# sapeirone/EgoPack

Hardware: AMD Instinct MI355X
Metric: clip-seqs/sec training, AR+LTA+PNR multi-task (higher is better)
Workload: dtype bf16; 1 GPU; MTL pre-train AR+LTA+PNR (BASELINE config 3): per GPU B=64 seqs/task x T=32 nodes, 3x1536-d Omnivore-shaped features, H=1024, TRN hidden 1024 (dropout 0.5), depth 3, k=1, Adam; graph mode, fused backbone pass; global_batch=192, parallelism=dp1, trainable_params=25003272, capture=one graph, input=resident in HBM before the timed region, master_weights=f32, mode=bf16, activations=bf16

## Files before the change

### egopack_amd/csrc/gemm.hip

```cpp
#include <type_traits>

#include "common.h"

namespace egk {

typedef __attribute__((ext_vector_type(4))) float f32x4;
typedef __attribute__((ext_vector_type(8))) __bf16 bf16x8;
typedef unsigned short bf16_t;

constexpr int BM = 128, BN = 128, ROWB = 128;
constexpr int NTHREADS = 256;

constexpr int MAXSRC = 6;
struct GemmArgs {
    int M, N;
    int nsrc;
    int K[MAXSRC];
    const void* A[MAXSRC];
    const void* B[MAXSRC];
    long long lda[MAXSRC], ldb[MAXSRC];
    int a_vec, b_vec;
    void* C;
    long long ldc;
    int c_vec, c_bf16;
    int accumulate, act;
    float alpha;
    const float* bias;
    const void* residual;
    long long ldr;
    int r_vec, r_bf16;
    int splitk;
    float* ws;
    int tiles_m, tiles_n;
    int group_m;
    float* dbias;
    float* ws_bias;
    int rows_epilogue;
    int st_mode, st_nseg;
    const int* st_seg_ptr;
    double* st_ws;
    const void* st_x;
    long long st_ldx;
    const float* st_stats;
    const float* st_w;
    const float* st_b;
    float st_slope;
};

__device__ __forceinline__ void tile_of_virtual(const GemmArgs& g, int v, int& z, int& tm, int& tn) {
    const int tiles = g.tiles_m * g.tiles_n;
    z = v / tiles;
    const int t = v - z * tiles;
    const int gsz = g.group_m * g.tiles_n;
    const int grp = t / gsz, first = grp * g.group_m;
    const int rows = min(g.group_m, g.tiles_m - first);
    const int rr = t - grp * gsz;
    tm = first + rr % rows;
    tn = rr / rows;
}
__device__ __forceinline__ void tile_of(const GemmArgs& g, int bid, int& z, int& tm, int& tn) {
    const int tiles = g.tiles_m * g.tiles_n, nwg = tiles * g.splitk;
    const int xcd = bid & 7, q = nwg >> 3, r = nwg & 7;
    const int v = (xcd < r ? xcd * (q + 1) : r * (q + 1) + (xcd - r) * q) + (bid >> 3);
    z = v / tiles;
    const int t = v - z * tiles;
    const int gsz = g.group_m * g.tiles_n;
    const int grp = t / gsz, first = grp * g.group_m;
    const int rows = min(g.group_m, g.tiles_m - first);
    const int rr = t - grp * gsz;
    tm = first + rr % rows;
    tn = rr / rows;
}

template <int KT>
__device__ __forceinline__ void source_of(const GemmArgs& g, int t, int& src, int& tt) {
    src = 0;
    tt = t;
    while (src + 1 < g.nsrc) {
        const int n = (g.K[src] + KT - 1) / KT;
// ... 370 lines not shown
                const float* xp = (const float*)g.st_x + (long long)m * g.st_ldx + n;
                const float4 x0 = *reinterpret_cast<const float4*>(xp), x1 = *reinterpret_cast<const float4*>(xp + 4);
                xv[0] = x0.x; xv[1] = x0.y; xv[2] = x0.z; xv[3] = x0.w; xv[4] = x1.x; xv[5] = x1.y; xv[6] = x1.z; xv[7] = x1.w;
            }
            float a1 = 0.f, a2 = 0.f;
#pragma unroll
            for (int t = 0; t < 8; ++t) {
                const float xh = (xv[t] - mu) * ri;
                const float pre = xh * lw[t] + lb[t];
                const float dxh = o[t] * (pre > 0.f ? 1.f : g.st_slope) * lw[t];
                a1 += dxh;
                a2 += dxh * xh;
            }
            sa[rel][0] += a1;
            sa[rel][1] += a2;
        }
    }
    if constexpr (ST) if (st_mode) {
        __shared__ double st_red_static[MBW == 1 ? 4 : 1][4];
        double (*st_red)[4] = st_red_static;
        if constexpr (MBW == 2) st_red = reinterpret_cast<double (*)[4]>(lds + 32 * NI * MBW * 512);
        double v4[4] = {(double)sa[0][0], (double)sa[0][1], (double)sa[1][0], (double)sa[1][1]};
#pragma unroll
        for (int q = 0; q < 4; ++q)
#pragma unroll
            for (int o_ = 32; o_ > 0; o_ >>= 1) v4[q] += __shfl_xor(v4[q], o_, 64);
        if ((tid & 63) == 0) {
#pragma unroll
            for (int q = 0; q < 4; ++q) st_red[tid >> 6][q] = v4[q];
        }
        __syncthreads();
        if (tid < g.st_nseg * 2) {
            const int sg = tid >> 1, k = tid & 1, rel = sg - s0;
            double t_ = 0.0;
            if (rel == 0 || rel == 1) {
                t_ = (st_red[0][rel * 2 + k] + st_red[1][rel * 2 + k]) + (st_red[2][rel * 2 + k] + st_red[3][rel * 2 + k]);
                if constexpr (MBW == 2)
                    t_ += (st_red[4][rel * 2 + k] + st_red[5][rel * 2 + k]) + (st_red[6][rel * 2 + k] + st_red[7][rel * 2 + k]);
            }
            g.st_ws[((long long)st_tile * g.st_nseg + sg) * 2 + k] = t_;
        }
    }
}

template <bool BF16C, bool TA, bool TB, typename AT, typename BT>
__global__ __launch_bounds__(NTHREADS) void gemm_kernel(const GemmArgs g) {
    __shared__ __attribute__((aligned(16))) unsigned char lds[2 * BM * ROWB];
    unsigned char* ldsA = lds;
    unsigned char* ldsB = lds + BM * ROWB;
    constexpr int KT = BF16C ? 64 : 32;
    constexpr bool A16 = sizeof(AT) == 2, B16 = sizeof(BT) == 2;

    const int nwg = g.tiles_m * g.tiles_n;
    int bid = blockIdx.x;
    {
        const int xcd = bid & 7, q = nwg >> 3, r = nwg & 7;
        bid = (xcd < r ? xcd * (q + 1) : r * (q + 1) + (xcd - r) * q) + (bid >> 3);
    }
    const int tm = bid / g.tiles_n, tn = bid % g.tiles_n;
    const int m0 = tm * BM, n0 = tn * BN;

    const int nkt = total_tiles(g, KT);
    const int z = blockIdx.y;
    const int per = (nkt + g.splitk - 1) / g.splitk;
    const int t_begin = z * per, t_end = min(nkt, t_begin + per);

// ... 173 lines not shown
            const int L = wall - WG;
            OperandCursor<TRA, PA> la;
            OperandCursor<TRB, PB> lb;
            int lsrc = -1;
            auto lissue = [&](int i, int stage) {
                const int t = t_begin + i;
                int src, tt;
                source_of<KT>(g, t, src, tt);
                if (src != lsrc) {
                    const int k0 = tt * KT;
                    la.init((const bf16_t*)g.A[src], g.lda[src], g.M, m0, k0, L * PA, lane, 1);
                    lb.init((const bf16_t*)g.B[src], g.ldb[src], g.N, n0, k0, L * PB, lane, 1);
                    lsrc = src;
                }
                unsigned char* sbase = ring + stage * STAGE;
                la.issue(sbase, L * PA);
                lb.issue(sbase + IMG_A, L * PB);
            };
#pragma unroll
            for (int p = 0; p < NSTAGE - 1; ++p)
                if (p < nt) lissue(p, p);
            for (int it = 0; it < rounds; ++it) {
                const int later = min(NSTAGE - 2, nt - 1 - it);
                if (later >= 2) asm volatile("s_waitcnt vmcnt(%0)" ::"n"(2 * (PA + PB)) : "memory");
                else if (later == 1) asm volatile("s_waitcnt vmcnt(%0)" ::"n"(PA + PB) : "memory");
                else asm volatile("s_waitcnt vmcnt(0)" ::: "memory");
                __builtin_amdgcn_s_barrier();
                if (it + NSTAGE - 1 < nt) lissue(it + NSTAGE - 1, (it + NSTAGE - 1) % NSTAGE);
            }
            return;
        }
    }

    f32x4 acc[NI][4];
#pragma unroll
    for (int i = 0; i < NI; ++i)
#pragma unroll
        for (int j = 0; j < 4; ++j) acc[i][j] = f32x4{0.f, 0.f, 0.f, 0.f};

    const unsigned lds_base = (unsigned)(size_t)(lds_void_t*)ring;
    const unsigned rm_sw = (unsigned)((lg ^ ((lr >> 1) & 7)) << 4);
    const unsigned a_rm = (unsigned)((wm * 16 * NI + lr) * ROWB) + rm_sw;
    const unsigned b_rm = (unsigned)((wn * 64 + lr) * ROWB) + rm_sw;
    const int tq = (lane & 15) >> 2, tp = lane & 3;
    const unsigned tr_row = (unsigned)((8 * lg + tq) * 256 + (tp & 1) * 8);
    const unsigned tr_f = (unsigned)(2 * tq + 8 * (lg & 1));
    unsigned a_tr[4], b_tr[4];
#pragma unroll
    for (int i = 0; i < 4; ++i) {
        a_tr[i] = (unsigned)((wm >> 1) * IMG) + tr_row + ((((unsigned)((wm & 1) * 8 + 2 * i + (tp >> 1))) ^ tr_f) << 4);
        b_tr[i] = tr_row + ((((unsigned)(wn * 8 + 2 * i + (tp >> 1))) ^ tr_f) << 4);
    }

    const bool do_bias = TRA && g.dbias != nullptr && tn == 0;
    float bsum[8] = {0.f, 0.f, 0.f, 0.f, 0.f, 0.f, 0.f, 0.f};
    const int bcc = tid & 15, bkg = (tid & 255) >> 4;
    const int bsub = MB == 2 ? (tid >> 8) : 0;

    uint4 a0[4], a1[4], b0[4], b1[4];
    if constexpr (LW == 0) {
#pragma unroll
        for (int p = 0; p < NSTAGE - 1; ++p)
            if (p < nt) issue(p, p);
    }
    for (int it = 0; it < rounds; ++it) {
        if constexpr (LW == 0) {
// ... 100 lines not shown
                    const unsigned wv[4] = {bz[r].x, bz[r].y, bz[r].z, bz[r].w};
#pragma unroll
                    for (int e = 0; e < 4; ++e) {
                        bsum[2 * e] += __uint_as_float(wv[e] << 16);
                        bsum[2 * e + 1] += __uint_as_float(wv[e] & 0xffff0000u);
                    }
                }
            }
        }
    }
#ifdef EGK_GEMM_STAMPS
    const unsigned long long ps_loop = __builtin_amdgcn_s_memtime();
#endif
    if constexpr (TRA) {
        if (g.dbias != nullptr && tn == 0) {
            __syncthreads();
            float* red = reinterpret_cast<float*>(lds);
            const int slot = MB == 2 ? bsub : grp;
#pragma unroll
            for (int e = 0; e < 8; ++e) red[(slot * 16 + bkg) * 128 + bcc * 8 + e] = bsum[e];
            __syncthreads();
            if (tid < 128 * MB && m0 + tid < g.M) {
                const int q0 = MB == 2 ? (tid >> 7) * 16 : 0, nq = MB == 2 ? 16 : 16 * KG;
                float t = 0.f;
                for (int q = 0; q < nq; ++q) t += red[(q0 + q) * 128 + (tid & 127)];
                if (g.splitk > 1) g.ws_bias[(long long)z * g.M + m0 + tid] = t;
                else g.dbias[m0 + tid] += t;
            }
            __syncthreads();
        }
    }
    if constexpr (KG == 1) {
        if constexpr (MB == 1) {
            if (epilogue_rows_ok(g)) gemm_epilogue_rows<NI>(g, acc, lds, m0, n0, wm, wn, lr, lg, z, tid, tm * g.tiles_n + tn);
            else gemm_epilogue<NI, 4>(g, acc, m0, n0, wm * 16 * NI, wn * 64, lr, lg, z);
        } else if constexpr (NI == 3) {
            static_assert(NSTAGE * STAGE >= 192 * 512 + 256, "the rows epilogue stages the whole tile (+ the wave partials) in the ring");
            if (epilogue_rows_ok(g)) gemm_epilogue_rows<NI, true, 2>(g, acc, lds, m0, n0, wm, wn, lr, lg, z, tid, tm * g.tiles_n + tn);
            else gemm_epilogue<NI, 4>(g, acc, m0, n0, wm * 16 * NI, wn * 64, lr, lg, z);
        } else {
            gemm_epilogue<NI, 4>(g, acc, m0, n0, wm * 16 * NI, wn * 64, lr, lg, z);
        }
    } else if constexpr (NI == 4 || NI == 2) {
        constexpr int HF = NI / 2;
        __syncthreads();
        f32x4* xch = reinterpret_cast<f32x4*>(lds);
        f32x4* mine_out = xch + ((grp * 4 + w) * (HF * 4)) * 64 + lane;
        const f32x4* theirs = xch + (((1 - grp) * 4 + w) * (HF * 4)) * 64 + lane;
        f32x4 half[HF][4];
        if (grp == 0) {
#pragma unroll
            for (int i = 0; i < HF; ++i)
#pragma unroll
                for (int j = 0; j < 4; ++j) mine_out[(i * 4 + j) * 64] = acc[HF + i][j];
        } else {
#pragma unroll
            for (int i = 0; i < HF; ++i)
#pragma unroll
                for (int j = 0; j < 4; ++j) mine_out[(i * 4 + j) * 64] = acc[i][j];
        }
        __syncthreads();
        if (grp == 0) {
#pragma unroll
            for (int i = 0; i < HF; ++i)
#pragma unroll
                for (int j = 0; j < 4; ++j) half[i][j] = acc[i][j] + theirs[(i * 4 + j) * 64];
        } else {
#pragma unroll
            for (int i = 0; i < HF; ++i)
#pragma unroll
                for (int j = 0; j < 4; ++j) half[i][j] = theirs[(i * 4 + j) * 64] + acc[HF + i][j];
// ... 23 lines not shown
    float o[4] = {s4.x * g.alpha, s4.y * g.alpha, s4.z * g.alpha, s4.w * g.alpha};
    if (g.accumulate) {
        const float4 c = *reinterpret_cast<const float4*>((const float*)g.C + (long long)m * g.ldc + n);
        o[0] += c.x; o[1] += c.y; o[2] += c.z; o[3] += c.w;
    }
    if (g.bias) {
#pragma unroll
        for (int t = 0; t < 4; ++t) o[t] += g.bias[n + t];
    }
    if (g.act == EGK_ACT_RELU) {
#pragma unroll
        for (int t = 0; t < 4; ++t) o[t] = fmaxf(o[t], 0.f);
    }
    if (g.residual) {
        if (g.r_bf16) {
            const uint2 r = *reinterpret_cast<const uint2*>((const bf16_t*)g.residual + (long long)m * g.ldr + n);
            o[0] += __uint_as_float(r.x << 16); o[1] += __uint_as_float(r.x & 0xffff0000u);
            o[2] += __uint_as_float(r.y << 16); o[3] += __uint_as_float(r.y & 0xffff0000u);
        } else {
            const float4 r = *reinterpret_cast<const float4*>((const float*)g.residual + (long long)m * g.ldr + n);
            o[0] += r.x; o[1] += r.y; o[2] += r.z; o[3] += r.w;
        }
    }
    if (g.c_bf16) {
        uint2 pk;
        pk.x = (unsigned)f32_to_bf16(o[0]) | ((unsigned)f32_to_bf16(o[1]) << 16);
        pk.y = (unsigned)f32_to_bf16(o[2]) | ((unsigned)f32_to_bf16(o[3]) << 16);
        *reinterpret_cast<uint2*>((bf16_t*)g.C + (long long)m * g.ldc + n) = pk;
    } else {
        *reinterpret_cast<float4*>((float*)g.C + (long long)m * g.ldc + n) = make_float4(o[0], o[1], o[2], o[3]);
    }
}

template <int NSTAGE, bool TRA, bool TRB, int KG, int MB, int NI = 4, bool F16 = false, int LW = 0>
__global__ __launch_bounds__(NTHREADS * KG * MB + 64 * LW) void gemm_pipe_kernel(const GemmArgs g) {
    gemm_pipe_body<NSTAGE, TRA, TRB, KG, MB, NI, false, F16, LW>(g, blockIdx.x);
}

constexpr int MAX_GROUPS = 8;
struct GemmGroup {
    GemmArgs p[MAX_GROUPS];
    int packed, count, total;
};
template <int NSTAGE, bool TRA, bool TRB, int KG, int MB, int NI = 4, bool F16 = false, int LW = 0>
__global__ __launch_bounds__(NTHREADS * KG * MB + 64 * LW) void gemm_pipe_group_kernel(const GemmGroup gg) {
    if (gg.packed) {
        const int lin = blockIdx.x, xcd = lin & 7, slot = lin >> 3;
        const int q = gg.total >> 3, r = gg.total & 7;
        if (slot >= q + (xcd < r ? 1 : 0)) return;
        int v = (xcd < r ? xcd * (q + 1) : r * (q + 1) + (xcd - r) * q) + slot;
        int pi = 0;
        for (; pi + 1 < gg.count; ++pi) {
            const int t = gg.p[pi].tiles_m * gg.p[pi].tiles_n;
            if (v < t) break;
            v -= t;
        }
        gemm_pipe_body<NSTAGE, TRA, TRB, KG, MB, NI, true, F16, LW>(gg.p[pi], v);
        return;
    }
    const GemmArgs& g = gg.p[blockIdx.y];
    if ((int)blockIdx.x >= g.tiles_m * g.tiles_n * g.splitk) return;
    gemm_pipe_body<NSTAGE, TRA, TRB, KG, MB, NI, false, F16, LW>(g, blockIdx.x);
}


template <bool TR, int FIRST, int S, int CNT = 4>
__device__ __forceinline__ void read_frags4(uint4 (&dst)[4], unsigned st, unsigned rm, const unsigned* tr) {
    if constexpr (TR) {
#pragma unroll
        for (int i = 0; i < CNT; ++i) {
            const unsigned ad = st + tr[FIRST + i];
            uint2 lo, hi;
            asm volatile("ds_read_b64_tr_b16 %0, %1 offset:%2" : "=v"(lo) : "v"(ad), "n"(S * 8192));
            asm volatile("ds_read_b64_tr_b16 %0, %1 offset:%2" : "=v"(hi) : "v"(ad), "n"(S * 8192 + 1024));
            dst[i] = make_uint4(lo.x, lo.y, hi.x, hi.y);
        }
    } else {
        const unsigned ad = S ? ((st + rm) ^ 64u) : (st + rm);
// ... 304 lines not shown
        asm volatile("s_waitcnt lgkmcnt(0)" ::: "memory");
        __builtin_amdgcn_sched_barrier(0);
        read_step32<TRA, 1, NI>(a1, stA, a_rm, a_tr);
        read_step32<TRB, 1, 4>(b1, stB, b_rm, b_tr);
        mfma_step(a0, b0);
        asm volatile("s_waitcnt lgkmcnt(0)" ::: "memory");
        __builtin_amdgcn_sched_barrier(0);
        mfma_step(a1, b1);
        if constexpr (TRA) {
            if (do_bias) {
#pragma unroll
                for (int r = 0; r < 4; ++r)
#pragma unroll
                    for (int e = 0; e < 4; ++e) bsum[e] += bz[r][e];
            }
        }
    }
    if constexpr (TRA) {
        if (g.dbias != nullptr && tn == 0) {
            __syncthreads();
            float* red = reinterpret_cast<float*>(lds);
#pragma unroll
            for (int e = 0; e < 4; ++e) red[bkg * 128 + bcc * 4 + e] = bsum[e];
            __syncthreads();
            if (tid < 128 && m0 + tid < g.M) {
                float t = 0.f;
                for (int q = 0; q < 8; ++q) t += red[q * 128 + tid];
                if (g.splitk > 1) g.ws_bias[(long long)z * g.M + m0 + tid] = t;
                else g.dbias[m0 + tid] += t;
            }
            __syncthreads();
        }
    }
    if (epilogue_rows_ok(g)) gemm_epilogue_rows<NI>(g, acc, lds, m0, n0, wm, wn, lr, lg, z, tid, tm * g.tiles_n + tn);
    else gemm_epilogue<NI, 4>(g, acc, m0, n0, wm * 16 * NI, wn * 64, lr, lg, z);
}

template <bool TRA, bool TRB, int NI = 4>
__global__ __launch_bounds__(NTHREADS) void gemm_pipe_f32_kernel(const GemmArgs g) {
    gemm_pipe_f32_body<TRA, TRB, NI, false>(g, blockIdx.x);
}

template <bool TRA, bool TRB>
__global__ __launch_bounds__(NTHREADS) void gemm_pipe_f32_group_kernel(const GemmGroup gg) {
    const int lin = blockIdx.x, xcd = lin & 7, slot = lin >> 3;
    const int q = gg.total >> 3, r = gg.total & 7;
    if (slot >= q + (xcd < r ? 1 : 0)) return;
    int v = (xcd < r ? xcd * (q + 1) : r * (q + 1) + (xcd - r) * q) + slot;
    int pi = 0;
    for (; pi + 1 < gg.count; ++pi) {
        const int t = gg.p[pi].tiles_m * gg.p[pi].tiles_n;
        if (v < t) break;
        v -= t;
    }
    gemm_pipe_f32_body<TRA, TRB, 4, true>(gg.p[pi], v);
}

__global__ __launch_bounds__(256) void gemm_splitk_reduce(const GemmArgs g) {
    const long long total = (long long)g.M * g.N;
    const bool vec4 = (g.N & 3) == 0 && g.c_vec && (!g.residual || g.r_vec);
    if (vec4) {
        const int gpr = g.N >> 2;
        const long long groups = (long long)g.M * gpr;
        for (long long q = (long long)blockIdx.x * blockDim.x + threadIdx.x; q < groups; q += (long long)gridDim.x * blockDim.x) {
            const int m = (int)(q / gpr), n = (int)(q - (long long)m * gpr) * 4;
            splitk_finish_group(g, m, n, total);
        }
    } else {
        for (long long idx = (long long)blockIdx.x * blockDim.x + threadIdx.x; idx < total;
             idx += (long long)gridDim.x * blockDim.x) {
            const int m = (int)(idx / g.N), n = (int)(idx % g.N);
            float s = 0.f;
            for (int z = 0; z < g.splitk; ++z) s += g.ws[(long long)z * total + idx];
            float o = s * g.alpha;
            if (g.accumulate) o += ((const float*)g.C)[(long long)m * g.ldc + n];
            if (g.bias) o += g.bias[n];
            if (g.act == EGK_ACT_RELU) o = fmaxf(o, 0.f);
            if (g.residual)
                o += g.r_bf16 ? bf16_to_f32(((const bf16_t*)g.residual)[(long long)m * g.ldr + n])
                              : ((const float*)g.residual)[(long long)m * g.ldr + n];
            if (g.c_bf16) ((bf16_t*)g.C)[(long long)m * g.ldc + n] = f32_to_bf16(o);
            else ((float*)g.C)[(long long)m * g.ldc + n] = o;
        }
    }
    if (g.dbias && g.ws_bias)
        for (long long m = (long long)blockIdx.x * blockDim.x + threadIdx.x; m < g.M; m += (long long)gridDim.x * blockDim.x) {
            float t = 0.f;
            for (int z = 0; z < g.splitk; ++z) t += g.ws_bias[(long long)z * g.M + m];
            g.dbias[m] += t;
        }
}

static inline bool aligned16(const void* p) { return (reinterpret_cast<uintptr_t>(p) & 15) == 0; }

template <bool BF16C, typename AT, typename BT>
static void launch_layout(const egk_gemm_desc* d, dim3 grid, hipStream_t s, const GemmArgs& g) {
    dim3 block(NTHREADS);
    if (!d->transA && !d->transB) hipLaunchKernelGGL((gemm_kernel<BF16C, false, false, AT, BT>), grid, block, 0, s, g);
    else if (!d->transA && d->transB) hipLaunchKernelGGL((gemm_kernel<BF16C, false, true, AT, BT>), grid, block, 0, s, g);
    else if (d->transA && d->transB) hipLaunchKernelGGL((gemm_kernel<BF16C, true, true, AT, BT>), grid, block, 0, s, g);
    else hipLaunchKernelGGL((gemm_kernel<BF16C, true, false, AT, BT>), grid, block, 0, s, g);
}

}

using namespace egk;

static int g_use_pipe = 1;
static constexpr double REDUCE_FIXED_US = 3.5;
static int g_r192_loaders = 1;
static int g_tt_tall = 1;
static bool g_lds_attr_set = false;
template <int NS, bool TA, bool TB, int KG, int MB = 1>
static void set_lds_attr() {
    (void)hipFuncSetAttribute((const void*)egk::gemm_pipe_kernel<NS, TA, TB, KG, MB>, hipFuncAttributeMaxDynamicSharedMemorySize,
                              NS * KG * (MB + 1) * 16384);
}
static void ensure_lds_attr() {
    if (g_lds_attr_set) return;
    set_lds_attr<2, false, false, 1>(); set_lds_attr<2, false, true, 1>(); set_lds_attr<2, true, true, 1>(); set_lds_attr<2, true, false, 1>();
    set_lds_attr<2, false, false, 2>(); set_lds_attr<2, false, true, 2>(); set_lds_attr<2, true, true, 2>(); set_lds_attr<2, true, false, 2>();
    (void)hipFuncSetAttribute((const void*)egk::gemm_pipe_kernel<2, false, false, 1, 1, 2>, hipFuncAttributeMaxDynamicSharedMemorySize, 65536);
    (void)hipFuncSetAttribute((const void*)egk::gemm_pipe_kernel<2, false, true, 1, 1, 2>, hipFuncAttributeMaxDynamicSharedMemorySize, 65536);
    (void)hipFuncSetAttribute((const void*)egk::gemm_pipe_kernel<2, false, false, 1, 1, 3>, hipFuncAttributeMaxDynamicSharedMemorySize, 65536);
    (void)hipFuncSetAttribute((const void*)egk::gemm_pipe_kernel<2, false, true, 1, 1, 3>, hipFuncAttributeMaxDynamicSharedMemorySize, 65536);
    (void)hipFuncSetAttribute((const void*)egk::gemm_big_kernel<false, false>, hipFuncAttributeMaxDynamicSharedMemorySize, 131072);
    (void)hipFuncSetAttribute((const void*)egk::gemm_big_kernel<false, true>, hipFuncAttributeMaxDynamicSharedMemorySize, 131072);
    (void)hipFuncSetAttribute((const void*)egk::gemm_big_kernel<true, true>, hipFuncAttributeMaxDynamicSharedMemorySize, 131072);
    (void)hipFuncSetAttribute((const void*)egk::gemm_big_kernel<true, false>, hipFuncAttributeMaxDynamicSharedMemorySize, 131072);
    (void)hipFuncSetAttribute((const void*)egk::gemm_big_kernel<false, false, 8, 6>, hipFuncAttributeMaxDynamicSharedMemorySize, 131072);
    (void)hipFuncSetAttribute((const void*)egk::gemm_big_kernel<false, true, 8, 6>, hipFuncAttributeMaxDynamicSharedMemorySize, 131072);
    (void)hipFuncSetAttribute((const void*)egk::gemm_pipe_group_kernel<2, false, false, 1, 1, 2>, hipFuncAttributeMaxDynamicSharedMemorySize, 65536);
    (void)hipFuncSetAttribute((const void*)egk::gemm_pipe_group_kernel<2, false, true, 1, 1, 2>, hipFuncAttributeMaxDynamicSharedMemorySize, 65536);
    (void)hipFuncSetAttribute((const void*)egk::gemm_pipe_group_kernel<2, false, false, 1, 1, 3>, hipFuncAttributeMaxDynamicSharedMemorySize, 65536);
    (void)hipFuncSetAttribute((const void*)egk::gemm_pipe_group_kernel<2, false, true, 1, 1, 3>, hipFuncAttributeMaxDynamicSharedMemorySize, 65536);
    (void)hipFuncSetAttribute((const void*)egk::gemm_pipe_group_kernel<2, false, false, 1, 1>, hipFuncAttributeMaxDynamicSharedMemorySize, 65536);
    (void)hipFuncSetAttribute((const void*)egk::gemm_pipe_group_kernel<2, false, false, 1, 1, 4, true>, hipFuncAttributeMaxDynamicSharedMemorySize, 65536);
    (void)hipFuncSetAttribute((const void*)egk::gemm_pipe_group_kernel<2, false, true, 1, 1>, hipFuncAttributeMaxDynamicSharedMemorySize, 65536);
    (void)hipFuncSetAttribute((const void*)egk::gemm_pipe_group_kernel<2, true, true, 1, 1>, hipFuncAttributeMaxDynamicSharedMemorySize, 131072);
    (void)hipFuncSetAttribute((const void*)egk::gemm_pipe_group_kernel<2, true, true, 2, 1>, hipFuncAttributeMaxDynamicSharedMemorySize, 131072);
    (void)hipFuncSetAttribute((const void*)egk::gemm_pipe_group_kernel<3, true, true, 1, 2>, hipFuncAttributeMaxDynamicSharedMemorySize, 3 * 49152);
    (void)hipFuncSetAttribute((const void*)egk::gemm_pipe_group_kernel<3, false, false, 1, 2, 3, false, 4>, hipFuncAttributeMaxDynamicSharedMemorySize, 3 * 40960);
    (void)hipFuncSetAttribute((const void*)egk::gemm_pipe_group_kernel<3, false, true, 1, 2, 3, false, 4>, hipFuncAttributeMaxDynamicSharedMemorySize, 3 * 40960);
    (void)hipFuncSetAttribute((const void*)egk::gemm_pipe_group_kernel<2, false, false, 2, 1>, hipFuncAttributeMaxDynamicSharedMemorySize, 131072);
    (void)hipFuncSetAttribute((const void*)egk::gemm_pipe_group_kernel<2, false, true, 2, 1>, hipFuncAttributeMaxDynamicSharedMemorySize, 131072);
    (void)hipFuncSetAttribute((const void*)egk::gemm_pipe_f32_kernel<false, false>, hipFuncAttributeMaxDynamicSharedMemorySize, 65536);
    (void)hipFuncSetAttribute((const void*)egk::gemm_pipe_f32_kernel<false, true>, hipFuncAttributeMaxDynamicSharedMemorySize, 65536);
    (void)hipFuncSetAttribute((const void*)egk::gemm_pipe_f32_kernel<true, true>, hipFuncAttributeMaxDynamicSharedMemorySize, 65536);
    (void)hipFuncSetAttribute((const void*)egk::gemm_pipe_f32_kernel<true, false>, hipFuncAttributeMaxDynamicSharedMemorySize, 65536);
    (void)hipFuncSetAttribute((const void*)egk::gemm_pipe_f32_group_kernel<false, false>, hipFuncAttributeMaxDynamicSharedMemorySize, 65536);
    (void)hipFuncSetAttribute((const void*)egk::gemm_pipe_f32_group_kernel<false, true>, hipFuncAttributeMaxDynamicSharedMemorySize, 65536);
    (void)hipFuncSetAttribute((const void*)egk::gemm_pipe_f32_group_kernel<true, true>, hipFuncAttributeMaxDynamicSharedMemorySize, 65536);
    (void)hipFuncSetAttribute((const void*)egk::gemm_pipe_f32_kernel<false, false, 3>, hipFuncAttributeMaxDynamicSharedMemorySize, 65536);
    (void)hipFuncSetAttribute((const void*)egk::gemm_pipe_f32_kernel<false, true, 3>, hipFuncAttributeMaxDynamicSharedMemorySize, 65536);
    (void)hipFuncSetAttribute((const void*)egk::gemm_pipe_kernel<3, false, false, 1, 2, 3>, hipFuncAttributeMaxDynamicSharedMemorySize, 3 * 40960);
    (void)hipFuncSetAttribute((const void*)egk::gemm_pipe_kernel<3, false, true, 1, 2, 3>, hipFuncAttributeMaxDynamicSharedMemorySize, 3 * 40960);
    (void)hipFuncSetAttribute((const void*)egk::gemm_pipe_kernel<3, false, false, 1, 2, 3, false, 4>, hipFuncAttributeMaxDynamicSharedMemorySize, 3 * 40960);
    (void)hipFuncSetAttribute((const void*)egk::gemm_pipe_kernel<3, false, true, 1, 2, 3, false, 4>, hipFuncAttributeMaxDynamicSharedMemorySize, 3 * 40960);
    (void)hipFuncSetAttribute((const void*)egk::gemm_pipe_kernel<2, false, false, 2, 1, 2>, hipFuncAttributeMaxDynamicSharedMemorySize, 4 * 24576);
    (void)hipFuncSetAttribute((const void*)egk::gemm_pipe_kernel<2, false, true, 2, 1, 2>, hipFuncAttributeMaxDynamicSharedMemorySize, 4 * 24576);
    g_lds_attr_set = true;
}
extern "C" int egk_gemm_set_pipeline(int32_t on) {
    const int prev = g_use_pipe;
    if (on == 870 || on == 871) { g_r192_loaders = on - 870; return prev; }
    if (on == 850 || on == 851) { g_tt_tall = on - 850; return prev; }
    if (on < 0 || on >= 20) return -1;
    g_use_pipe = on;
    return prev;
}

extern "C" int egk_gemm_splitk(int32_t M, int32_t N, int32_t K, int32_t compute) {
    const int KT = compute == EGK_COMPUTE_BF16 ? 64 : 32;
    const int tiles = cdiv(M, BM) * cdiv(N, BN);
    const int nkt = cdiv(K, KT);
    if (compute != EGK_COMPUTE_BF16) {
        if (nkt < 8) return 1;
        const double mn = (double)M * N / 1048576.0;
        const long long t96 = (long long)cdiv(M, 96) * cdiv(N, BN);
        auto rounds = [&](int s_) {
            const double r128 = (double)cdiv((long long)tiles * s_, 256), r96 = 0.75 * cdiv(t96 * s_, 256);
            return r128 < r96 ? r128 : r96;
        };
        int best = 1;
        double best_cost = rounds(1) * nkt * 1.9;
        for (int s = 2; s <= 16 && nkt / s >= 4; ++s) {
            const double cost = rounds(s) * cdiv(nkt, s) * 1.9 + 3.5 + 1.5 * s * mn;
            if (cost < 0.93 * best_cost) { best_cost = cost; best = s; }
        }
        return best;
    }
    if (tiles > 128 || nkt < 4) return 1;
    const double mn = (double)M * N / 1048576.0;
    int best = 1;
    double best_cost = 6.5 + 0.45 * nkt;
    for (int s = 2; s <= 16 && tiles * s <= 256 && nkt / s >= 2; s *= 2) {
        const double cost = 6.5 + 0.45 * cdiv(nkt, s) + REDUCE_FIXED_US + 1.5 * s * mn;
// ... 77 lines not shown
    hipStream_t s = (hipStream_t)stream;

    GemmArgs g;
    g.M = d->M; g.N = d->N;
    const int ea = a16 ? 8 : 4, eb = b16 ? 8 : 4;
    SourceInfo src;
    {
        const int rc = fill_sources(d, g, ea, eb, src, "egk_gemm");
        if (rc) return rc;
    }
    g.C = d->C; g.ldc = d->ldc;
    g.c_bf16 = d->c_dtype == EGK_BF16;
    g.c_vec = g.c_bf16 ? ((reinterpret_cast<uintptr_t>(g.C) & 7) == 0 && g.ldc % 4 == 0) : (aligned16(g.C) && g.ldc % 4 == 0);
    g.accumulate = d->accumulate; g.act = d->act; g.alpha = d->alpha;
    g.bias = d->bias; g.residual = d->residual; g.ldr = d->ldr;
    g.r_bf16 = d->r_dtype == EGK_BF16;
    g.r_vec = g.residual && (g.r_bf16 ? ((reinterpret_cast<uintptr_t>(g.residual) & 7) == 0 && g.ldr % 4 == 0)
                                      : (aligned16(g.residual) && g.ldr % 4 == 0));
    g.splitk = d->splitk > 1 ? d->splitk : 1;
    g.ws = (float*)d->ws;
    if (g.splitk > 1)
        EGK_REQUIRE(g.ws && d->ws_bytes >= (int64_t)g.splitk * d->M * d->N * 4, "egk_gemm: split-K workspace too small");
    g.tiles_m = cdiv(g.M, BM); g.tiles_n = cdiv(g.N, BN);
    g.dbias = nullptr; g.ws_bias = nullptr;
    g.group_m = 1;
    g.rows_epilogue = 1;
    g.st_mode = d->st_mode; g.st_nseg = d->st_nseg; g.st_seg_ptr = d->st_seg_ptr; g.st_ws = (double*)d->st_ws;
    g.st_x = d->st_x; g.st_ldx = d->st_ldx; g.st_stats = d->st_stats; g.st_w = d->st_w; g.st_b = d->st_b; g.st_slope = d->st_slope;
    if (d->st_mode) {
        EGK_REQUIRE(d->st_mode == 1 || d->st_mode == 2, "egk_gemm: st_mode must be 0, 1 or 2");
        EGK_REQUIRE(d->st_nseg >= 1 && d->st_nseg <= 16 && d->st_seg_ptr && (query_blocks || d->st_ws), "egk_gemm: st_* segments / workspace");
        EGK_REQUIRE(d->st_mode == 1 || (d->st_x && d->st_stats && d->st_w && d->st_b), "egk_gemm: st_mode 2 needs x, stats, w, b");
    }
    if (query_blocks) *query_blocks = 0;
    const long long K = src.k_total;
    const double flops = 2.0 * d->M * d->N * K;
    const double bytes = (a16 ? 2.0 : 4.0) * ((double)d->M * K + (double)d->N * K) + (g.c_bf16 ? 2.0 : 4.0) * d->M * d->N;
    const int bf = d->compute == EGK_COMPUTE_BF16;
    const int layout = d->transA ? (d->transB ? 2 : 3) : (d->transB ? 1 : 0);
    const double slab_bytes = d->splitk > 1 ? ((double)d->splitk + 1.0) * d->M * d->N * 4.0 : 0.0;

    const bool pipe_ok = bf && a16 && g_use_pipe && src.all_k64 && K > 0 && src.all_vec;
    const bool single = d->K2 == 0 && d->n_extra == 0;
    bool all_k32 = K > 0;
    for (int i = 0; i < g.nsrc; ++i) all_k32 = all_k32 && (g.K[i] % 32 == 0);
    const bool pipe32_ok = !bf && !a16 && g_use_pipe && all_k32 && src.all_vec;
    const bool bias_fused = (pipe_ok || pipe32_ok) && d->dbias && d->transA && single;
    if (d->dbias) {
        EGK_REQUIRE(d->transA && single, "egk_gemm: dbias needs the dW form (transA, single K source)");
        const int64_t slab = g.splitk > 1 ? (int64_t)g.splitk * d->M * d->N * 4 : 0;
        const int64_t need = bias_fused ? slab + (g.splitk > 1 ? (int64_t)g.splitk * d->M * 4 : 0)
                                        : slab + (int64_t)egk_colsum_ws_len(d->K1, d->M) * 4;
        EGK_REQUIRE(d->ws && d->ws_bytes >= need, "egk_gemm: workspace too small for dbias (%lld bytes needed)", (long long)need);
        if (bias_fused) {
            g.dbias = d->dbias;
            g.ws_bias = g.splitk > 1 ? (float*)((char*)d->ws + slab) : nullptr;
        } else if (!query_blocks) {
            const int rc = egk_colsum(stream, d->A1, d->lda1, d->K1, d->M, d->dbias, 1, (float*)((char*)d->ws + slab), d->a_dtype);
            if (rc) return rc;
        }
    }
    if (pipe_ok) {
        ensure_lds_attr();
        dim3 pblock(NTHREADS);
        const int nwg128 = g.tiles_m * g.tiles_n * g.splitk;
        const int nkt_slab = cdiv(K / 64, g.splitk);
// ... 202 lines not shown
    EGK_REQUIRE(f32p || (d->a_dtype == EGK_BF16 && d->b_dtype == EGK_BF16 && d->compute == EGK_COMPUTE_BF16),
                "egk_gemm_grouped: bf16 operands on the bf16 MFMA path, or f32 operands on the exact-f32 path");
    EGK_REQUIRE(d->splitk <= 1, "egk_gemm_grouped: no split-K in a grouped launch");
    EGK_REQUIRE(!(d->accumulate && d->c_dtype != EGK_F32), "egk_gemm_grouped: accumulate needs an f32 C");
    EGK_REQUIRE(d->C, "egk_gemm_grouped: null pointer");
    EGK_REQUIRE(!d->dbias || (d->transA && d->K2 == 0 && d->n_extra == 0), "egk_gemm_grouped: dbias needs the dW form (transA, single K source)");
    g.M = d->M; g.N = d->N;
    SourceInfo src;
    {
        const int rc = fill_sources(d, g, f32p ? 4 : 8, f32p ? 4 : 8, src, "egk_gemm_grouped");
        if (rc) return rc;
    }
    if (f32p) {
        for (int i = 0; i < g.nsrc; ++i) EGK_REQUIRE(g.K[i] % 32 == 0, "egk_gemm_grouped: f32 K sources must be multiples of 32");
    } else {
        EGK_REQUIRE(src.all_k64, "egk_gemm_grouped: K sources must be multiples of 64");
    }
    EGK_REQUIRE(src.all_vec, "egk_gemm_grouped: operand rows must be 16-byte aligned");
    g.C = d->C; g.ldc = d->ldc;
    g.c_bf16 = d->c_dtype == EGK_BF16;
    g.c_vec = g.c_bf16 ? ((reinterpret_cast<uintptr_t>(g.C) & 7) == 0 && g.ldc % 4 == 0) : (aligned16(g.C) && g.ldc % 4 == 0);
    g.accumulate = d->accumulate; g.act = d->act; g.alpha = d->alpha;
    g.bias = d->bias; g.residual = d->residual; g.ldr = d->ldr;
    g.r_bf16 = d->r_dtype == EGK_BF16;
    g.r_vec = g.residual && (g.r_bf16 ? ((reinterpret_cast<uintptr_t>(g.residual) & 7) == 0 && g.ldr % 4 == 0)
                                      : (aligned16(g.residual) && g.ldr % 4 == 0));
    g.splitk = 1;
    g.ws = nullptr;
    g.dbias = d->dbias; g.ws_bias = nullptr;
    g.rows_epilogue = 1;
    g.st_mode = 0; g.st_nseg = 0; g.st_seg_ptr = nullptr; g.st_ws = nullptr; g.st_x = nullptr; g.st_ldx = 0;
    g.st_stats = nullptr; g.st_w = nullptr; g.st_b = nullptr; g.st_slope = 0.f;
    EGK_REQUIRE(d->st_mode == 0, "egk_gemm_grouped: no segment statistics in a grouped launch");
    return 0;
}

extern "C" int egk_gemm_grouped(egk_stream_t stream, const egk_gemm_desc* descs, int32_t count) {
    EGK_REQUIRE(descs != nullptr && count >= 1 && count <= MAX_GROUPS, "egk_gemm_grouped: 1 .. %d problems", MAX_GROUPS);
    if (count == 1) return egk_gemm(stream, descs);
    hipStream_t s = (hipStream_t)stream;
    GemmGroup gg;
    const bool ta = descs[0].transA != 0, tb = descs[0].transB != 0;
    const bool f32g = descs[0].compute == EGK_COMPUTE_F32;
    const bool f16 = descs[0].op_f16 != 0;
    EGK_REQUIRE(!f16 || (!ta && !tb && !f32g), "egk_gemm_grouped: op_f16 takes row-major 16-bit operands");
    double flops = 0, bytes = 0;
    long long t128 = 0, t96 = 0, t64 = 0, t256 = 0, t192 = 0;
    int min_nkt = 1 << 30, any_extra = 0;
    for (int i = 0; i < count; ++i) {
        const egk_gemm_desc* d = descs + i;
        EGK_REQUIRE((d->transA != 0) == ta && (d->transB != 0) == tb, "egk_gemm_grouped: the problems must share one layout");
        EGK_REQUIRE((d->compute == EGK_COMPUTE_F32) == f32g, "egk_gemm_grouped: the problems must share one compute type");
        EGK_REQUIRE((d->op_f16 != 0) == f16, "egk_gemm_grouped: the problems must agree on op_f16");
        EGK_REQUIRE(!f16 || (!d->st_mode && !d->dbias && d->n_extra == 0), "egk_gemm_grouped: op_f16 has no statistics / bias-gradient epilogue");
        const int rc = fill_group_args(d, gg.p[i]);
        if (rc) return rc;
        int K = d->K1 + d->K2;
        for (int x = 0; x < d->n_extra; ++x) K += d->xK[x];
        flops += 2.0 * d->M * d->N * K;
        bytes += 2.0 * ((double)d->M * K + (double)d->N * K) + (gg.p[i].c_bf16 ? 2.0 : 4.0) * d->M * d->N;
        const int tn = cdiv(d->N, BN);
        t128 += (long long)cdiv(d->M, 128) * tn; t96 += (long long)cdiv(d->M, 96) * tn; t64 += (long long)cdiv(d->M, 64) * tn;
        t256 += (long long)cdiv(d->M, 256) * tn;
        t192 += (long long)cdiv(d->M, 192) * tn;
        any_extra |= d->n_extra > 0;
        min_nkt = K / 64 < min_nkt ? K / 64 : min_nkt;
// ... 92 lines not shown
```

Before: 149,400 clip-seqs/s.

## Add specialized rows epilogue with mode-dispatched store loops and prefetched per-column params

Adds a new GEMM rows epilogue that computes a bitmask of epilogue features, switches to compile-time specialized store loops for common mode combinations, batches all residual/accumulate loads ahead of the LDS reads, and prefetches bias and layer-norm weights before the main loop. It also adds minimum-waves hints to launch_bounds for the pipe and f32 kernels. The aim is to cut epilogue branching and load latency and to raise occupancy. In exchange it increases code size and register pressure, and the launch_bounds hints can force spills.

```diff
diff --git a/egopack_amd/csrc/gemm.hip b/egopack_amd/csrc/gemm.hip
--- a/egopack_amd/csrc/gemm.hip
+++ b/egopack_amd/csrc/gemm.hip
@@ -45,6 +45,7 @@
     const float* st_w;
     const float* st_b;
     float st_slope;
+    int epi;
 };
 
 __device__ __forceinline__ void tile_of_virtual(const GemmArgs& g, int v, int& z, int& tm, int& tn) {
@@ -481,6 +482,310 @@
         __syncthreads();
         if (tid < g.st_nseg * 2) {
             const int sg = tid >> 1, k = tid & 1, rel = sg - s0;
+            double t_ = 0.0;
+            if (rel == 0 || rel == 1) {
+                t_ = (st_red[0][rel * 2 + k] + st_red[1][rel * 2 + k]) + (st_red[2][rel * 2 + k] + st_red[3][rel * 2 + k]);
+                if constexpr (MBW == 2)
+                    t_ += (st_red[4][rel * 2 + k] + st_red[5][rel * 2 + k]) + (st_red[6][rel * 2 + k] + st_red[7][rel * 2 + k]);
+            }
+            g.st_ws[((long long)st_tile * g.st_nseg + sg) * 2 + k] = t_;
+        }
+    }
+}
+
+enum : unsigned { RM_ACC = 1, RM_BIAS = 2, RM_RELU = 4, RM_RES16 = 8, RM_RES32 = 16, RM_CB = 32, RM_ST1 = 64, RM_ST2 = 128, RM_SLAB = 256 };
+
+struct RowsPre {
+    unsigned mode;
+    int s0, s_split;
+    float mu[2], ri[2];
+    float bias[8], lw[8], lb[8];
+};
+
+template <bool ST, bool W = true>
+__device__ __forceinline__ void rows_prefetch(const GemmArgs& g, int m0, int n0, int tid, RowsPre& P) {
+    unsigned mode = RM_SLAB;
+    if (g.splitk == 1) {
+        mode = (g.accumulate ? RM_ACC : 0u) | (g.bias ? RM_BIAS : 0u) | (g.act == EGK_ACT_RELU ? RM_RELU : 0u) |
+               (g.residual ? (g.r_bf16 ? RM_RES16 : RM_RES32) : 0u) | (g.c_bf16 ? RM_CB : 0u);
+        if (ST && g.st_mode) mode |= g.st_mode == 2 ? RM_ST2 : RM_ST1;
+    }
+    P.mode = mode;
+    P.s0 = 0;
+    P.s_split = 0x7fffffff;
+    P.mu[0] = P.mu[1] = P.ri[0] = P.ri[1] = 0.f;
+#pragma unroll
+    for (int t = 0; t < 8; ++t) P.bias[t] = P.lw[t] = P.lb[t] = 0.f;
+    const int n = n0 + (tid & 15) * 8;
+    const bool cols = n < g.N;
+    if ((mode & RM_BIAS) && cols) {
+        const float4 b0 = *reinterpret_cast<const float4*>(g.bias + n), b1 = *reinterpret_cast<const float4*>(g.bias + n + 4);
+        P.bias[0] = b0.x; P.bias[1] = b0.y; P.bias[2] = b0.z; P.bias[3] = b0.w; P.bias[4] = b1.x; P.bias[5] = b1.y; P.bias[6] = b1.z; P.bias[7] = b1.w;
+    }
+    if (mode & (RM_ST1 | RM_ST2)) {
+        int s0 = 0;
+        while (s0 + 1 < g.st_nseg && m0 >= g.st_seg_ptr[s0 + 1]) ++s0;
+        if (s0 + 1 < g.st_nseg) P.s_split = g.st_seg_ptr[s0 + 1];
+        P.s0 = s0;
+        if (mode & RM_ST2) {
+            P.mu[0] = g.st_stats[s0 * 2]; P.ri[0] = g.st_stats[s0 * 2 + 1];
+            if (s0 + 1 < g.st_nseg) { P.mu[1] = g.st_stats[s0 * 2 + 2]; P.ri[1] = g.st_stats[s0 * 2 + 3]; }
+            if (W && cols) {
+                const float4 w0 = *reinterpret_cast<const float4*>(g.st_w + n), w1 = *reinterpret_cast<const float4*>(g.st_w + n + 4);
+                const float4 c0 = *reinterpret_cast<const float4*>(g.st_b + n), c1 = *reinterpret_cast<const float4*>(g.st_b + n + 4);
+                P.lw[0] = w0.x; P.lw[1] = w0.y; P.lw[2] = w0.z; P.lw[3] = w0.w; P.lw[4] = w1.x; P.lw[5] = w1.y; P.lw[6] = w1.z; P.lw[7] = w1.w;
+                P.lb[0] = c0.x; P.lb[1] = c0.y; P.lb[2] = c0.z; P.lb[3] = c0.w; P.lb[4] = c1.x; P.lb[5] = c1.y; P.lb[6] = c1.z; P.lb[7] = c1.w;
+            }
+        }
+    }
+}
+
+__device__ __forceinline__ void rows_prefetch_w(const GemmArgs& g, int n0, int tid, RowsPre& P) {
+    const int n = n0 + (tid & 15) * 8;
+    if ((P.mode & RM_ST2) && n < g.N) {
+        const float4 w0 = *reinterpret_cast<const float4*>(g.st_w + n), w1 = *reinterpret_cast<const float4*>(g.st_w + n + 4);
+        const float4 c0 = *reinterpret_cast<const float4*>(g.st_b + n), c1 = *reinterpret_cast<const float4*>(g.st_b + n + 4);
+        P.lw[0] = w0.x; P.lw[1] = w0.y; P.lw[2] = w0.z; P.lw[3] = w0.w; P.lw[4] = w1.x; P.lw[5] = w1.y; P.lw[6] = w1.z; P.lw[7] = w1.w;
+        P.lb[0] = c0.x; P.lb[1] = c0.y; P.lb[2] = c0.z; P.lb[3] = c0.w; P.lb[4] = c1.x; P.lb[5] = c1.y; P.lb[6] = c1.z; P.lb[7] = c1.w;
+    }
+}
+
+struct RowsDesc {
+    int M, N;
+    unsigned mode;
+    float alpha, slope;
+    char* C;
+    const char* R;
+    const char* X;
+    float* ws;
+    long long ldc, ldr, ldx;
+};
+
+typedef __attribute__((ext_vector_type(4))) unsigned u32x4;
+typedef const __attribute__((address_space(1))) f32x4* gload_f32x4;
+typedef const __attribute__((address_space(1))) u32x4* gload_u32x4;
+typedef __attribute__((address_space(1))) f32x4* gstore_f32x4;
+typedef __attribute__((address_space(1))) u32x4* gstore_u32x4;
+
+__device__ __forceinline__ void unpack_bf16x8(const u32x4& r, float (&f)[8]) {
+#pragma unroll
+    for (int t = 0; t < 4; ++t) {
+        f[2 * t] = __uint_as_float(r[t] << 16);
+        f[2 * t + 1] = __uint_as_float(r[t] & 0xffff0000u);
+    }
+}
+
+struct RowLoads {
+    f32x4 c0, c1, r0, r1, x0, x1;
+    u32x4 rh, xh;
+};
+
+__device__ __forceinline__ void rows_load(const RowsDesc& D, unsigned mode, long long mc, int n, RowLoads& L) {
+    if (mode & RM_ACC) {
+        const gload_f32x4 cp = (gload_f32x4)(D.C + (mc * D.ldc + n) * 4);
+        L.c0 = cp[0]; L.c1 = cp[1];
+    }
+    if (mode & RM_RES16) L.rh = *(gload_u32x4)(D.R + (mc * D.ldr + n) * 2);
+    if (mode & RM_RES32) {
+        const gload_f32x4 rp = (gload_f32x4)(D.R + (mc * D.ldr + n) * 4);
+        L.r0 = rp[0]; L.r1 = rp[1];
+    }
+    if (mode & RM_ST2) {
+        if (mode & RM_CB) L.xh = *(gload_u32x4)(D.X + (mc * D.ldx + n) * 2);
+        else {
+            const gload_f32x4 xp = (gload_f32x4)(D.X + (mc * D.ldx + n) * 4);
+            L.x0 = xp[0]; L.x1 = xp[1];
+        }
+    }
+}
+
+__device__ __forceinline__ void rows_finish(const RowsDesc& D, const RowsPre& P, unsigned mode, const f32x4& lo, const f32x4& hi,
+                                            const RowLoads& L, int m, int n, int z, float (&sa)[2][2]) {
+#pragma clang fp contract(off)
+    const bool ok = m < D.M;
+    float o[8] = {lo[0], lo[1], lo[2], lo[3], hi[0], hi[1], hi[2], hi[3]};
+    if (mode & RM_SLAB) {
+        if (ok) {
+            const gstore_f32x4 p = (gstore_f32x4)(reinterpret_cast<char*>(D.ws) + (((long long)z * D.M + m) * D.N + n) * 4);
+            p[0] = lo; p[1] = hi;
+        }
+        return;
+    }
+#pragma unroll
+    for (int t = 0; t < 8; ++t) o[t] *= D.alpha;
+    if (mode & RM_ACC)
+#pragma unroll
+        for (int t = 0; t < 4; ++t) { o[t] += L.c0[t]; o[4 + t] += L.c1[t]; }
+    if (mode & RM_BIAS)
+#pragma unroll
+        for (int t = 0; t < 8; ++t) o[t] += P.bias[t];
+    if (mode & RM_RELU)
+#pragma unroll
+        for (int t = 0; t < 8; ++t) o[t] = fmaxf(o[t], 0.f);
+    if (mode & RM_RES16) {
+        float r[8];
+        unpack_bf16x8(L.rh, r);
+#pragma unroll
+        for (int t = 0; t < 8; ++t) o[t] += r[t];
+    }
+    if (mode & RM_RES32)
+#pragma unroll
+        for (int t = 0; t < 4; ++t) { o[t] += L.r0[t]; o[4 + t] += L.r1[t]; }
+    if (mode & RM_CB) {
+        u32x4 pk;
+#pragma unroll
+        for (int t = 0; t < 4; ++t) pk[t] = (unsigned)f32_to_bf16(o[2 * t]) | ((unsigned)f32_to_bf16(o[2 * t + 1]) << 16);
+        if (ok) *(gstore_u32x4)(D.C + ((long long)m * D.ldc + n) * 2) = pk;
+        if (mode & (RM_ST1 | RM_ST2)) unpack_bf16x8(pk, o);
+    } else if (ok) {
+        const gstore_f32x4 cp = (gstore_f32x4)(D.C + ((long long)m * D.ldc + n) * 4);
+        cp[0] = f32x4{o[0], o[1], o[2], o[3]};
+        cp[1] = f32x4{o[4], o[5], o[6], o[7]};
+    }
+    if (!(mode & (RM_ST1 | RM_ST2))) return;
+    const bool rel = m >= P.s_split;
+    float a1 = 0.f, a2 = 0.f;
+    if (mode & RM_ST1) {
+#pragma unroll
+        for (int t = 0; t < 8; ++t) {
+            a1 += o[t];
+            a2 += o[t] * o[t];
+        }
+    } else {
+        const float mu = rel ? P.mu[1] : P.mu[0], ri = rel ? P.ri[1] : P.ri[0];
+        float xv[8];
+        if (mode & RM_CB) unpack_bf16x8(L.xh, xv);
+        else
+#pragma unroll
+            for (int t = 0; t < 4; ++t) { xv[t] = L.x0[t]; xv[4 + t] = L.x1[t]; }
+#pragma unroll
+        for (int t = 0; t < 8; ++t) {
+            const float xh = (xv[t] - mu) * ri;
+            const float pre = __builtin_fmaf(xh, P.lw[t], P.lb[t]);
+            const float dxh = o[t] * (pre > 0.f ? 1.f : D.slope) * P.lw[t];
+            a1 += dxh;
+            a2 += dxh * xh;
+        }
+    }
+    sa[0][0] = (ok && !rel) ? sa[0][0] + a1 : sa[0][0];
+    sa[0][1] = (ok && !rel) ? sa[0][1] + a2 : sa[0][1];
+    sa[1][0] = (ok && rel) ? sa[1][0] + a1 : sa[1][0];
+    sa[1][1] = (ok && rel) ? sa[1][1] + a2 : sa[1][1];
+    asm volatile("" : "+v"(sa[0][0]), "+v"(sa[0][1]), "+v"(sa[1][0]), "+v"(sa[1][1]));
+}
+
+template <int NI, int MBW, bool GEN, unsigned F>
+__device__ __forceinline__ void rows_store_loop(const RowsDesc& D, const RowsPre& P, const float* stage, int m0, int n, int z, int tid,
+                                                float (&sa)[2][2]) {
+    constexpr int NIT = 2 * NI;
+    const int c8 = tid & 15, last = D.M - 1;
+    int r0 = tid >> 4;
+    asm volatile("; rows loop %1" : "+v"(r0) : "n"(GEN ? 0xfff : F));
+    if constexpr (GEN) {
+#pragma unroll 1
+        for (int it = 0; it < NIT; ++it) {
+            const int row = it * (16 * MBW) + r0;
+            const f32x4 lo = *reinterpret_cast<const f32x4*>(stage + row * 128 + (((2 * c8) ^ (row & 15)) << 2));
+            const f32x4 hi = *reinterpret_cast<const f32x4*>(stage + row * 128 + (((2 * c8 + 1) ^ (row & 15)) << 2));
+            RowLoads L;
+            rows_load(D, D.mode, min(m0 + row, last), n, L);
+            rows_finish(D, P, D.mode, lo, hi, L, m0 + row, n, z, sa);
+        }
+    } else {
+        constexpr int CH = (F & RM_ST2) ? 1 : NI;
+        RowLoads L[NIT];
+#pragma unroll
+        for (int it = 0; it < NIT; ++it) rows_load(D, F, min(m0 + it * (16 * MBW) + r0, last), n, L[it]);
+#pragma unroll
+        for (int c0 = 0; c0 < NIT; c0 += CH) {
+            __builtin_amdgcn_sched_barrier(0);
+            f32x4 lo[CH], hi[CH];
+#pragma unroll
+            for (int k = 0; k < CH; ++k) {
+                const int row = (c0 + k) * (16 * MBW) + r0;
+                lo[k] = *reinterpret_cast<const f32x4*>(stage + row * 128 + (((2 * c8) ^ (row & 15)) << 2));
+                hi[k] = *reinterpret_cast<const f32x4*>(stage + row * 128 + (((2 * c8 + 1) ^ (row & 15)) << 2));
+            }
+            if constexpr ((F & (RM_ACC | RM_RES16 | RM_RES32 | RM_ST2)) != 0)
+                if (c0 == 0) __builtin_amdgcn_s_waitcnt(0x0F70);
+#pragma unroll
+            for (int k = 0; k < CH; ++k)
+                rows_finish(D, P, F, lo[k], hi[k], L[c0 + k], m0 + (c0 + k) * (16 * MBW) + r0, n, z, sa);
+        }
+    }
+}
+
+template <int NI, bool ST = true, int MBW = 1, bool PRE = false>
+__device__ __forceinline__ void gemm_epilogue_rows_fast(const GemmArgs& g, const f32x4 (&acc)[NI][4], unsigned char* lds, int m0, int n0,
+                                                        int wm, int wn, int lr, int lg, int z, int tid, int st_tile, RowsPre& P) {
+    RowsDesc D;
+    {
+        int M = g.M, N = g.N;
+        unsigned mode = PRE ? P.mode : 0u;
+        float alpha = g.alpha, slope = g.st_slope;
+        char* C = reinterpret_cast<char*>(g.C);
+        const char* R = reinterpret_cast<const char*>(g.residual);
+        const char* X = reinterpret_cast<const char*>(g.st_x);
+        float* ws = g.ws;
+        long long ldc = g.ldc, ldr = g.ldr, ldx = g.st_ldx;
+        asm volatile("" : "+s"(M), "+s"(N), "+s"(mode), "+s"(alpha), "+s"(slope));
+        asm volatile("" : "+s"(C), "+s"(R), "+s"(X), "+s"(ws));
+        asm volatile("" : "+s"(ldc), "+s"(ldr), "+s"(ldx));
+        D.M = M; D.N = N; D.mode = mode; D.alpha = alpha; D.slope = slope; D.C = C; D.R = R; D.X = X; D.ws = ws;
+        D.ldc = ldc; D.ldr = ldr; D.ldx = ldx;
+    }
+    __syncthreads();
+    float* stage = reinterpret_cast<float*>(lds);
+#pragma unroll
+    for (int i = 0; i < NI; ++i) {
+        const int row = wm * 16 * NI + i * 16 + lr;
+#pragma unroll
+        for (int j = 0; j < 4; ++j) {
+            const int slot = (wn * 16 + j * 4 + lg) ^ (row & 15);
+            *reinterpret_cast<f32x4*>(stage + row * 128 + slot * 4) = acc[i][j];
+        }
+    }
+    if constexpr (PRE) rows_prefetch_w(g, n0, tid, P);
+    else {
+        rows_prefetch<ST>(g, m0, n0, tid, P);
+        D.mode = P.mode;
+        asm volatile("" : "+s"(D.mode));
+    }
+    __syncthreads();
+    const int n = n0 + (tid & 15) * 8;
+    float sa[2][2] = {{0.f, 0.f}, {0.f, 0.f}};
+    if (n < D.N) {
+#define EGK_ROWS_CASE(F) case (F): rows_store_loop<NI, MBW, false, (F)>(D, P, stage, m0, n, z, tid, sa); break
+        switch (D.mode) {
+            EGK_ROWS_CASE(RM_CB);
+            EGK_ROWS_CASE(RM_CB | RM_BIAS);
+            EGK_ROWS_CASE(RM_CB | RM_BIAS | RM_RELU);
+            EGK_ROWS_CASE(RM_CB | RM_BIAS | RM_RES16);
+            EGK_ROWS_CASE(RM_CB | RM_BIAS | RM_ST1);
+            EGK_ROWS_CASE(RM_CB | RM_ST2);
+            EGK_ROWS_CASE(0u);
+            EGK_ROWS_CASE(RM_ACC);
+            EGK_ROWS_CASE(RM_SLAB);
+            default: rows_store_loop<NI, MBW, true, 0u>(D, P, stage, m0, n, z, tid, sa); break;
+        }
+#undef EGK_ROWS_CASE
+    }
+    if constexpr (ST) if (D.mode & (RM_ST1 | RM_ST2)) {
+        __shared__ double st_red_static[MBW == 1 ? 4 : 1][4];
+        double (*st_red)[4] = st_red_static;
+        if constexpr (MBW == 2) st_red = reinterpret_cast<double (*)[4]>(lds + 32 * NI * MBW * 512);
+        double v4[4] = {(double)sa[0][0], (double)sa[0][1], (double)sa[1][0], (double)sa[1][1]};
+#pragma unroll
+        for (int q = 0; q < 4; ++q)
+#pragma unroll
+            for (int o_ = 32; o_ > 0; o_ >>= 1) v4[q] += __shfl_xor(v4[q], o_, 64);
+        if ((tid & 63) == 0) {
+#pragma unroll
+            for (int q = 0; q < 4; ++q) st_red[tid >> 6][q] = v4[q];
+        }
+        __syncthreads();
+        if (tid < g.st_nseg * 2) {
+            const int sg = tid >> 1, k = tid & 1, rel = sg - P.s0;
             double t_ = 0.0;
             if (rel == 0 || rel == 1) {
                 t_ = (st_red[0][rel * 2 + k] + st_red[1][rel * 2 + k]) + (st_red[2][rel * 2 + k] + st_red[3][rel * 2 + k]);
@@ -720,6 +1025,12 @@
         }
     }
 
+    constexpr bool PRE = LW > 0 && KG == 1 && (MB == 1 || NI == 3);
+    RowsPre pre;
+    if constexpr (PRE) {
+        if (g.epi) rows_prefetch<true, false>(g, m0, n0, tid, pre);
+    }
+
     f32x4 acc[NI][4];
 #pragma unroll
     for (int i = 0; i < NI; ++i)
@@ -886,11 +1197,13 @@
     }
     if constexpr (KG == 1) {
         if constexpr (MB == 1) {
-            if (epilogue_rows_ok(g)) gemm_epilogue_rows<NI>(g, acc, lds, m0, n0, wm, wn, lr, lg, z, tid, tm * g.tiles_n + tn);
+            if (g.epi) gemm_epilogue_rows_fast<NI, true, 1, PRE>(g, acc, lds, m0, n0, wm, wn, lr, lg, z, tid, tm * g.tiles_n + tn, pre);
+            else if (epilogue_rows_ok(g)) gemm_epilogue_rows<NI>(g, acc, lds, m0, n0, wm, wn, lr, lg, z, tid, tm * g.tiles_n + tn);
             else gemm_epilogue<NI, 4>(g, acc, m0, n0, wm * 16 * NI, wn * 64, lr, lg, z);
         } else if constexpr (NI == 3) {
             static_assert(NSTAGE * STAGE >= 192 * 512 + 256, "the rows epilogue stages the whole tile (+ the wave partials) in the ring");
-            if (epilogue_rows_ok(g)) gemm_epilogue_rows<NI, true, 2>(g, acc, lds, m0, n0, wm, wn, lr, lg, z, tid, tm * g.tiles_n + tn);
+            if (g.epi) gemm_epilogue_rows_fast<NI, true, 2, PRE>(g, acc, lds, m0, n0, wm, wn, lr, lg, z, tid, tm * g.tiles_n + tn, pre);
+            else if (epilogue_rows_ok(g)) gemm_epilogue_rows<NI, true, 2>(g, acc, lds, m0, n0, wm, wn, lr, lg, z, tid, tm * g.tiles_n + tn);
             else gemm_epilogue<NI, 4>(g, acc, m0, n0, wm * 16 * NI, wn * 64, lr, lg, z);
         } else {
             gemm_epilogue<NI, 4>(g, acc, m0, n0, wm * 16 * NI, wn * 64, lr, lg, z);
@@ -980,8 +1293,9 @@
     }
 }
 
+constexpr int pipe_min_waves(int KG, int MB, int NI, int LW) { return (KG == 1 && MB == 1) ? (NI == 2 ? 3 : 2) : (LW > 0 ? 3 : 1); }
 template <int NSTAGE, bool TRA, bool TRB, int KG, int MB, int NI = 4, bool F16 = false, int LW = 0>
-__global__ __launch_bounds__(NTHREADS * KG * MB + 64 * LW) void gemm_pipe_kernel(const GemmArgs g) {
+__global__ __launch_bounds__(NTHREADS * KG * MB + 64 * LW, pipe_min_waves(KG, MB, NI, LW)) void gemm_pipe_kernel(const GemmArgs g) {
     gemm_pipe_body<NSTAGE, TRA, TRB, KG, MB, NI, false, F16, LW>(g, blockIdx.x);
 }
 
@@ -991,7 +1305,7 @@
     int packed, count, total;
 };
 template <int NSTAGE, bool TRA, bool TRB, int KG, int MB, int NI = 4, bool F16 = false, int LW = 0>
-__global__ __launch_bounds__(NTHREADS * KG * MB + 64 * LW) void gemm_pipe_group_kernel(const GemmGroup gg) {
+__global__ __launch_bounds__(NTHREADS * KG * MB + 64 * LW, pipe_min_waves(KG, MB, NI, LW)) void gemm_pipe_group_kernel(const GemmGroup gg) {
     if (gg.packed) {
         const int lin = blockIdx.x, xcd = lin & 7, slot = lin >> 3;
         const int q = gg.total >> 3, r = gg.total & 7;
@@ -1362,17 +1676,20 @@
             __syncthreads();
         }
     }
-    if (epilogue_rows_ok(g)) gemm_epilogue_rows<NI>(g, acc, lds, m0, n0, wm, wn, lr, lg, z, tid, tm * g.tiles_n + tn);
+    if (g.epi) {
+        RowsPre pre;
+        gemm_epilogue_rows_fast<NI>(g, acc, lds, m0, n0, wm, wn, lr, lg, z, tid, tm * g.tiles_n + tn, pre);
+    } else if (epilogue_rows_ok(g)) gemm_epilogue_rows<NI>(g, acc, lds, m0, n0, wm, wn, lr, lg, z, tid, tm * g.tiles_n + tn);
     else gemm_epilogue<NI, 4>(g, acc, m0, n0, wm * 16 * NI, wn * 64, lr, lg, z);
 }
 
 template <bool TRA, bool TRB, int NI = 4>
-__global__ __launch_bounds__(NTHREADS) void gemm_pipe_f32_kernel(const GemmArgs g) {
+__global__ __launch_bounds__(NTHREADS, 2) void gemm_pipe_f32_kernel(const GemmArgs g) {
     gemm_pipe_f32_body<TRA, TRB, NI, false>(g, blockIdx.x);
 }
 
 template <bool TRA, bool TRB>
-__global__ __launch_bounds__(NTHREADS) void gemm_pipe_f32_group_kernel(const GemmGroup gg) {
+__global__ __launch_bounds__(NTHREADS, 2) void gemm_pipe_f32_group_kernel(const GemmGroup gg) {
     const int lin = blockIdx.x, xcd = lin & 7, slot = lin >> 3;
     const int q = gg.total >> 3, r = gg.total & 7;
     if (slot >= q + (xcd < r ? 1 : 0)) return;
@@ -1439,6 +1756,7 @@
 static int g_use_pipe = 1;
 static constexpr double REDUCE_FIXED_US = 3.5;
 static int g_r192_loaders = 1;
+static int g_rows_fast = 1;
 static int g_tt_tall = 1;
 static bool g_lds_attr_set = false;
 template <int NS, bool TA, bool TB, int KG, int MB = 1>
@@ -1493,6 +1811,7 @@
 }
 extern "C" int egk_gemm_set_pipeline(int32_t on) {
     const int prev = g_use_pipe;
+    if (on == 890 || on == 891) { g_rows_fast = on - 890; return prev; }
     if (on == 870 || on == 871) { g_r192_loaders = on - 870; return prev; }
     if (on == 850 || on == 851) { g_tt_tall = on - 850; return prev; }
     if (on < 0 || on >= 20) return -1;
@@ -1636,6 +1955,7 @@
         EGK_REQUIRE(d->st_nseg >= 1 && d->st_nseg <= 16 && d->st_seg_ptr && (query_blocks || d->st_ws), "egk_gemm: st_* segments / workspace");
         EGK_REQUIRE(d->st_mode == 1 || (d->st_x && d->st_stats && d->st_w && d->st_b), "egk_gemm: st_mode 2 needs x, stats, w, b");
     }
+    g.epi = g_rows_fast && epilogue_rows_ok(g);
     if (query_blocks) *query_blocks = 0;
     const long long K = src.k_total;
     const double flops = 2.0 * d->M * d->N * K;
@@ -1904,6 +2224,7 @@
     g.st_mode = 0; g.st_nseg = 0; g.st_seg_ptr = nullptr; g.st_ws = nullptr; g.st_x = nullptr; g.st_ldx = 0;
     g.st_stats = nullptr; g.st_w = nullptr; g.st_b = nullptr; g.st_slope = 0.f;
     EGK_REQUIRE(d->st_mode == 0, "egk_gemm_grouped: no segment statistics in a grouped launch");
+    g.epi = g_rows_fast && epilogue_rows_ok(g);
     return 0;
 }
 
```

After: 154,900 clip-seqs/s, median of 6. +3.7%, better.
